# RhushabhVaghela/Custom-NVComp-with-ZSTD

Hardware: AMD Instinct MI355X
Metric: compress GB/s + ratio, 1 GB @ level 3, 64 KB chunks; libzstd round-trip OK (higher is better)
Workload: dtype u8; 1 GPU; C3: 16384 x 64 KiB chunks (1.00 GiB), level 3, independent frames; chunk_bytes=65536, chunks_total=16384, chunks_rank0=16384, level=3, parallelism=dp1 (contiguous chunk shards, RCCL all-gather of sizes inside the step), gathered_frame_bytes=388747049

## Files before the change

### custom-nvcomp-with-zstd_amd/csrc/zh_common.h

```cpp
#pragma once
#include <hip/hip_runtime.h>
#include <stdint.h>
#include "zstd_hip_params.h"
#include "zh_dict_ent.h"
#include "zh_block_plan.h"

typedef int16_t s16;
typedef int32_t s32;

#define ZH_STATS_LIT 0u
#define ZH_STATS_LL 256u
#define ZH_STATS_OF 320u
#define ZH_STATS_ML 384u
#define ZH_STATS_WORDS 448u

#define ZH_SEQ_CAP 13120u
#define ZH_SEQ_BYTES (ZH_SEQ_CAP * 8u)
#define ZH_K3_W 1u
#define ZH_K3_SEGS (21u * ZH_K3_W)
#define ZH_K3_SLOTS (64u * ZH_K3_W)
#define ZH_K3_RUN 16u
#define ZH_K3_SLOT(t, g) (3u * (g) + (t))
#define ZH_K3_TSTRIDE ZH_K3_RUN
#define ZH_K3_SEGLEN(nbseq) ((((nbseq) + ZH_K3_SEGS - 1u) / ZH_K3_SEGS + ZH_K3_RUN - 1u) & ~(ZH_K3_RUN - 1u))
#define ZH_K3_CODES(L) (2u * ZH_K3_SLOTS * (L))
#define ZH_K3_BYTES(nbseq) (3u * ZH_K3_SLOTS * ZH_K3_SEGLEN(nbseq))
#define ZH_LIT_BYTES (ZH_K3_BYTES(ZH_SEQ_CAP) > (u32)ZH_BLOCK_MAX ? ZH_K3_BYTES(ZH_SEQ_CAP) : (u32)ZH_BLOCK_MAX)
static_assert(3u * ZH_K3_SEGS <= ZH_K3_SLOTS, "one lane per (table, segment)");
#define ZH_META_BYTES 256u
#define ZH_FSE_BYTES 4096u
#define ZH_FSE_TAB_BYTES 3528u
#define ZH_FSE_FIELDS 3840u
static_assert(ZH_DENT_FSE_BYTES == ZH_FSE_TAB_BYTES, "the dictionary blob holds the tables in the hand-off layout");
#define ZH_WS_BLOCK_BYTES (ZH_SEQ_BYTES + ZH_LIT_BYTES + ZH_META_BYTES + ZH_FSE_BYTES)
enum : u32 {
  ZH_FT_STLL = 0, ZH_FT_STOF = 1024, ZH_FT_STML = 1536, ZH_FT_SYLL = 2560, ZH_FT_SYOF = 2848, ZH_FT_SYML = 3104,
  ZH_FF_NEED = 0,
  ZH_FF_NBSEQ = 1,
  ZH_FF_OP = 2,
  ZH_FF_BLK = 3,
  ZH_FF_LOGS = 4,
  ZH_FF_SLL = 5, ZH_FF_SOF = 6, ZH_FF_SML = 7,
};

#define ZH_DEEP_STG_BYTES (2u * ZH_BLOCK_MAX + 256u)
#define ZH_DEEP_SLOT_BYTES ((size_t)ZH_DEEP_STG_BYTES + 4u * 2u * ZH_BLOCK_MAX + 4u * ZH_BLOCK_MAX + 2u * 2u * ZH_BLOCK_MAX)
#define ZH_DEEP_SLOTS_MAX 256u
#define ZH_META_K1HIST 2u
#define ZH_K1_HIST_OFF 65536u
#define ZH_K1_HIST_WAVES 16u
static_assert(ZH_K1_HIST_OFF + ZH_K1_HIST_WAVES * 1024u <= ZH_LIT_BYTES, "K1 sub-histograms fit the literal area");

struct ZhWorkspace {
  u8 *base;
  u32 *ctr;
  const u16 *dtab;
  u32 dtab_P;
  const u32 *dd_prev;
  const u32 *dd_head;
  u32 dd_pre, dd_split;
  u8 *deep_slots;
  u32 deep_nslots;
  const ZhDictEnt *dent;
  u32 *stats;
  __device__ u64 *seq(u32 b) const { return (u64 *)(base + (size_t)b * ZH_WS_BLOCK_BYTES); }
  __device__ u8 *lits(u32 b) const { return base + (size_t)b * ZH_WS_BLOCK_BYTES + ZH_SEQ_BYTES; }
  __device__ u32 *meta(u32 b) const { return (u32 *)(base + (size_t)b * ZH_WS_BLOCK_BYTES + ZH_SEQ_BYTES + ZH_LIT_BYTES); }
  __device__ u32 *dbg(u32 b) const { return meta(b) + 4; }
  __device__ u8 *fse(u32 b) const { return base + (size_t)b * ZH_WS_BLOCK_BYTES + ZH_SEQ_BYTES + ZH_LIT_BYTES + ZH_META_BYTES; }
  __device__ u32 *fsef(u32 b) const { return (u32 *)(fse(b) + ZH_FSE_FIELDS); }
};

#define ZH_DTAB_MARGIN 256u

struct ZhClassRanges {
  u32 range[ZH_NCLASSES][2];
  u32 ctr[4];
};
#define ZH_RANGE_CTR_DEEP 3u

__host__ __device__ __forceinline__ u32 zh_k3_magic(u32 L) { return ((1u << 24) + L - 1u) / L; }
__device__ __forceinline__ u32 zh_k3_index(u32 e, u32 t, u32 L, u32 m) {
  u32 const g = __umulhi(e << 8, m), r = e - g * L;
  return ((r / ZH_K3_RUN) * ZH_K3_SLOTS + ZH_K3_SLOT(t, g)) * ZH_K3_RUN + (r & (ZH_K3_RUN - 1u));
}

#define ZH_DPP(v, ctrl, rmask) ((u32)__builtin_amdgcn_update_dpp(0, (int)(v), (ctrl), (rmask), 0xf, false))
__device__ __forceinline__ u32 wave_scan_incl(u32 v) {
  v += ZH_DPP(v, 0x111, 0xf);
  v += ZH_DPP(v, 0x112, 0xf);
  v += ZH_DPP(v, 0x114, 0xf);
  v += ZH_DPP(v, 0x118, 0xf);
  v += ZH_DPP(v, 0x142, 0xa);
  v += ZH_DPP(v, 0x143, 0xc);
  return v;
}
__device__ __forceinline__ u32 wave_scan_max_incl(u32 v) {
  v = max(v, ZH_DPP(v, 0x111, 0xf));
  v = max(v, ZH_DPP(v, 0x112, 0xf));
  v = max(v, ZH_DPP(v, 0x114, 0xf));
  v = max(v, ZH_DPP(v, 0x118, 0xf));
  v = max(v, ZH_DPP(v, 0x142, 0xa));
  v = max(v, ZH_DPP(v, 0x143, 0xc));
  return v;
}
__device__ __forceinline__ u32 wave_shr1(u32 v) { return ZH_DPP(v, 0x138, 0xf); }
__device__ __forceinline__ u32 wave_shl1(u32 v) { return ZH_DPP(v, 0x130, 0xf); }
__device__ __forceinline__ u32 lane_value(u32 v, u32 uniform_lane) { return (u32)__builtin_amdgcn_readlane((int)v, (int)uniform_lane); }
```

### custom-nvcomp-with-zstd_amd/csrc/zh_entropy.hip

```cpp
#include "zh_common.h"

namespace {

constexpr u32 K2_THREADS = 128;
constexpr u32 SW_WORDS = 184;

constexpr u32 OFF_SW = 0;
constexpr u32 OFF_HVAL = OFF_SW + 4 * SW_WORDS;
constexpr u32 OFF_HNB = OFF_HVAL + 2 * 256;
constexpr u32 OFF_MISC = OFF_HNB + 256;
constexpr u32 OFF_HIST = OFF_MISC + 4 * 64;
constexpr u32 OFF_HBUF = OFF_HIST + 4 * 256;
constexpr u32 OFF_SCR = OFF_HBUF + 768;
constexpr u32 OFF_U = OFF_SCR + 1024;
static_assert(OFF_U % 16 == 0, "alignment");
constexpr u32 OFF_NODES = OFF_U;
constexpr u32 U_HUF_END = OFF_NODES + 8 * 516;
constexpr u32 OFF_ST_LL = OFF_U;
constexpr u32 OFF_ST_OF = OFF_ST_LL + 1024;
constexpr u32 OFF_ST_ML = OFF_ST_OF + 512;
constexpr u32 OFF_SYM = OFF_ST_ML + 1024;
constexpr u32 SYM_OF = 36, SYM_ML = 68;
constexpr u32 OFF_TSYM = OFF_SYM + 976;
constexpr u32 OFF_NORM = OFF_TSYM + 512;
// ... 1278 lines not shown
          auto fse_candidate = [&](int &nv) {
            u32 nb1 = nbSeq;
            u32 const tl = fse_optimal_table_log(fseLog, nbSeq, mx, 2);
            u32 const lc = last_code[t];
            if (lane_value(c, lc) > 1) {
              if (lane == lc) c--;
              nb1--;
            }
            nv = fse_normalize_wave(norm, tl, c, nb1, mx, nb1 >= 2048, lane, scr->cumul);
            bmax = mx; blog = tl;
            return fse_write_ncount_wave(hbuf + hposw, nv, mx, tl, lane);
          };
          u32 fse_hs = 0;
          bool fse_done = false;
          if (dent && type != 1) {
            u32 const c0 = c, big = 0xFFFFFFFFu;
            u32 const dc = dent->cost[t][lane];
            u32 const costRep = __ballot(c0 != 0 && dc >= ZH_DENT_IMPOSSIBLE) ? big : wave_sum(c0 * dc);
            u32 costDef = big, costFse = big;
            if (defAllowed) costDef = wave_sum(c0 * fse_cost8(lane <= defMax ? (int)defNorm[lane] : 0, defLog));
            if (mostFrequent < nbSeq) {
              int nv;
              fse_hs = fse_candidate(nv);
              fse_done = true;
              if (fse_hs) costFse = (fse_hs << (3 + ZH_DENT_COST_SHIFT)) + wave_sum(c0 * fse_cost8(nv, blog));
            }
            if (costRep != big && costRep <= costDef && costRep <= costFse) type = 3;
            else if (costDef <= costFse) type = costDef != big ? 0 : type;
            else type = 2;
          }
          if (type == 3) {
            u32 const so = t == 0 ? ZH_FT_STLL : t == 1 ? ZH_FT_STOF : ZH_FT_STML, yo = t == 0 ? ZH_FT_SYLL : t == 1 ? ZH_FT_SYOF : ZH_FT_SYML;
            const u32 *const src = (const u32 *)(dent->fse + so);
            for (u32 i = lane; i < (t == 1 ? 128u : 256u); i += 64) ((u32 *)st)[i] = src[i];
            if (lane <= maxSym) sy[lane] = ((const FseSym *)(dent->fse + yo))[lane];
            logsw[t] = dent->logs[t];
          } else if (type == 1) {
            u32 const fc = first_code[t];
            if (lane == 0) {
              st[0] = 0; st[1] = 0;
              sy[fc].dNb = 0; sy[fc].dFS = 0;
              hbuf[hposw] = (u8)fc;
            }
            hposw++;
            logsw[t] = 0;
          } else if (type == 0) {
            if (lane <= defMax) norm[lane] = defNorm[lane];
            bmax = defMax; blog = defLog;
            logsw[t] = defLog;
          } else {
            int nv;
            if (!fse_done) fse_hs = fse_candidate(nv);
            hposw += fse_hs;
            logsw[t] = blog;
          }
          typesw |= type << (6 - 2 * t);
          wave_sync();
          if (type == 0 || type == 2) fse_build_ctable_par(st, sy, tsym, norm, bmax, blog, scr);
          wave_sync();
        }
        if (lane == 0) {
          misc[0] = hposw;
          misc[1] = typesw;
          misc[2] = logsw[0]; misc[3] = logsw[1]; misc[4] = logsw[2];
        }
      }
      wave_sync();
      hpos = misc[0];
      typesw_ = misc[1];
      logLL = misc[2]; logOF = misc[3]; logML = misc[4];
      ZH_STAMP(6);

      u8 *fz = ws.fse(b);
      {
        const u32 *sL = (const u32 *)stLL, *sO = (const u32 *)stOF, *sM = (const u32 *)stML;
        for (u32 i = lane; i < 256; i += 64) ((u32 *)(fz + ZH_FT_STLL))[i] = sL[i];
        for (u32 i = lane; i < 128; i += 64) ((u32 *)(fz + ZH_FT_STOF))[i] = sO[i];
        for (u32 i = lane; i < 256; i += 64) ((u32 *)(fz + ZH_FT_STML))[i] = sM[i];
        if (lane < 36) ((FseSym *)(fz + ZH_FT_SYLL))[lane] = symLL[lane];
        if (lane < 32) ((FseSym *)(fz + ZH_FT_SYOF))[lane] = symOF[lane];
        if (lane < 53) ((FseSym *)(fz + ZH_FT_SYML))[lane] = symML[lane];
      }
    }
    if (wave == 1 && lane == 0) xch[2] = nbSeq;
    }
    __syncthreads();
    if (xch[1] != 0) {
      u32 const h = (n / 2) & ~63u;
      if (wave == 0) copy_bytes(o, body0, d.src, h);
      else copy_bytes(o, body0 + h, d.src + h, n - h);
    } else if (u32 const ns = xch[2]; ns > 0) {
      u32 const k3L = ZH_K3_SEGLEN(ns), k3m = zh_k3_magic(k3L);
      u8 *const cb = ws.lits(b) + ZH_K3_CODES(k3L);
      for (u32 k0 = 16u * (lane + 64u * wave); k0 < ns; k0 += 16u * K2_THREADS) {
        u64 r[16];
#pragma unroll
        for (u32 q = 0; q < 16; q++) r[q] = k0 + q < ns ? seq[ns - 1 - (k0 + q)] : 0ull;
        u32 wl[4] = {0, 0, 0, 0}, wo[4] = {0, 0, 0, 0}, wm[4] = {0, 0, 0, 0};
#pragma unroll
        for (u32 q = 0; q < 16; q++) {
          u32 const ob = (u32)(r[q] >> 34) & 0x1FFFFu;
          wl[q >> 2] |= ((u32)(r[q] >> 51) & 63u) << (8 * (q & 3));
          wo[q >> 2] |= (ob ? highbit32(ob) : 0u) << (8 * (q & 3));
          wm[q >> 2] |= ((u32)(r[q] >> 57)) << (8 * (q & 3));
        }
        u32 const x0 = zh_k3_index(k0, 0, k3L, k3m);
        *(uint4 *)(cb + x0) = make_uint4(wl[0], wl[1], wl[2], wl[3]);
        *(uint4 *)(cb + x0 + ZH_K3_TSTRIDE) = make_uint4(wo[0], wo[1], wo[2], wo[3]);
        *(uint4 *)(cb + x0 + 2u * ZH_K3_TSTRIDE) = make_uint4(wm[0], wm[1], wm[2], wm[3]);
      }
    }
    if (wave == 1) {
      op = xch[0];
      early_raw = xch[1] != 0;
      if (!early_raw) {
        if (nbSeq < 128) { if (lane == 0) o.put(op, (u8)nbSeq); op += 1; }
        else if (nbSeq < ZH_LONGNBSEQ) { if (lane == 0) { o.put(op, (u8)((nbSeq >> 8) + 0x80)); o.put(op + 1, (u8)nbSeq); } op += 2; }
        else { if (lane == 0) { o.put(op, 0xFF); o.put(op + 1, (u8)(nbSeq - ZH_LONGNBSEQ)); o.put(op + 2, (u8)((nbSeq - ZH_LONGNBSEQ) >> 8)); } op += 3; }
        if (nbSeq > 0) {
          if (lane == 0) o.put(op, (u8)typesw_);
          op += 1;
          for (u32 i = lane; i < hpos; i += 64) o.put(op + i, hbuf[i]);
          op += hpos;
          u32 *ff = ws.fsef(b);
          if (lane == 0) {
            ff[ZH_FF_NBSEQ] = nbSeq; ff[ZH_FF_OP] = op; ff[ZH_FF_BLK] = blk;
            ff[ZH_FF_LOGS] = logLL | (logOF << 8) | (logML << 16);
            ff[ZH_FF_NEED] = 1;
          }
          handoff = true;
        }
      }
      if (early_raw) {
        u32 const hdr = last + (n << 3);
        if (lane == 0) { o.put(blk, (u8)hdr); o.put(blk + 1, (u8)(hdr >> 8)); o.put(blk + 2, (u8)(hdr >> 16)); }
        total = body0 + n;
      } else if (!handoff) {
        total = finish_block(d, o, blk, op, false);
      }
    }
  }
  ZH_STAMP(8);
#ifdef ZH_STAMPS
  if (lane == 0) {
    u32 *dbg = ws.dbg(b);
    if (wave == 0) { for (int k = 0; k < 4; k++) dbg[6 + k] = st[k]; dbg[42] = st[11]; }
    else { for (int k = 4; k < 9; k++) dbg[6 + k] = st[k]; dbg[17] = st[9]; dbg[18] = st[10]; dbg[19] = nseq_raw; }
  }
#endif
  if (wave == 1 && !handoff) write_status(d, b, total, item_size, item_status, blk_size);
}

constexpr u32 K3_SEGS = ZH_K3_SEGS;
constexpr u32 K3_W = ZH_K3_W;
constexpr u32 K3_OCC = 8;
constexpr u32 K3_WARM = 128;
constexpr u32 K3_WAVES = K3_W == 1 ? 4 : K3_W;
constexpr u32 K3_BPW = K3_WAVES / K3_W;
constexpr u32 K3_TAB_STRIDE = (ZH_FSE_TAB_BYTES + 15) & ~15u;
constexpr u32 K3_LDS = K3_BPW * K3_TAB_STRIDE + 64;
constexpr u32 K3_BATCH = 16;
constexpr u32 K3_TABW = ZH_FSE_TAB_BYTES / 4;

__device__ __forceinline__ void k3_chain(ZhWorkspace ws, u32 bb, u8 *smem, u32 lane, u32 *xw) {
#ifdef ZH_STAMPS
  u64 const k3pre = __builtin_amdgcn_s_memtime();
  u64 const k3rt0 = __builtin_amdgcn_s_memrealtime();
#endif
  u32 *ff = ws.fsef(bb);
  {
    const u32 *src = (const u32 *)ws.fse(bb);
    constexpr u32 NT = 64 * K3_W;
    u32 v[(K3_TABW + NT - 1) / NT];
#pragma unroll
    for (u32 q = 0; q < (K3_TABW + NT - 1) / NT; q++) v[q] = NT * q + lane < K3_TABW ? src[NT * q + lane] : 0u;
#pragma unroll
    for (u32 q = 0; q < (K3_TABW + NT - 1) / NT; q++)
      if (NT * q + lane < K3_TABW) ((u32 *)smem)[NT * q + lane] = v[q];
  }
  if constexpr (K3_W == 1) {
    __builtin_amdgcn_fence(__ATOMIC_SEQ_CST, "wavefront");
    __builtin_amdgcn_wave_barrier();
  } else {
    __syncthreads();
  }
  u32 const t = min(lane / K3_SEGS, 2u), g = lane - K3_SEGS * t;
  u32 const nbSeq = ff[ZH_FF_NBSEQ];
  const u16 *stT = (const u16 *)(smem + (t == 0 ? ZH_FT_STLL : t == 1 ? ZH_FT_STOF : ZH_FT_STML));
  const FseSym *syT = (const FseSym *)(smem + (t == 0 ? ZH_FT_SYLL : t == 1 ? ZH_FT_SYOF : ZH_FT_SYML));
  u32 const seglen = ZH_K3_SEGLEN(nbSeq), nk = seglen / K3_BATCH;
  u16 *const gst = (u16 *)ws.lits(bb);
  const u8 *const cbase = ws.lits(bb) + ZH_K3_CODES(seglen);
  u32 const ln = lane < 3 * K3_SEGS ? ZH_K3_SLOT(t, g) : lane, lnp = ZH_K3_SLOT(t, g - 1u);
  auto at = [&](u32 k, u32 slot) { return ((k * K3_BATCH / ZH_K3_RUN) * ZH_K3_SLOTS + slot) * ZH_K3_RUN + (k * K3_BATCH) % ZH_K3_RUN; };
  auto codes_at = [&](u32 k, u32 slot) { return *(const uint4 *)(cbase + at(k, slot)); };
  u32 const a = lane < 3 * K3_SEGS ? g * seglen : 3u * K3_SEGS * seglen;
  auto init_state = [&](u32 code) {
    FseSym const tr = syT[code];
    u32 const nb = (tr.dNb + (1u << 15)) >> 16;
    return (u32)stT[(((nb << 16) - tr.dNb) >> nb) + tr.dFS];
  };
  auto step = [&](u32 s, u32 code, bool live) {
    FseSym const tr = syT[code];
    u32 const nb = (s + tr.dNb) >> 16;
    u32 const nx = stT[min((s >> nb) + (u32)tr.dFS, 1023u)];
    return live ? nx : s;
  };
  u32 entry;
  if (a == 0) {
    entry = init_state(codes_at(0, ln).x & 63u);
  } else {
    constexpr u32 NW = K3_WARM / K3_BATCH;
    constexpr u32 CH = NW < 8u ? NW : 8u;
    static_assert(NW % CH == 0, "warm-up groups");
    u32 const kw = nk > NW ? nk - NW : 0u, ep = a - seglen;
    u32 s = stT[0];
#pragma unroll
    for (u32 j0 = 0; j0 < NW; j0 += CH) {
      uint4 cw[CH];
#pragma unroll
      for (u32 j = 0; j < CH; j++) cw[j] = kw + j0 + j < nk ? codes_at(kw + j0 + j, lnp) : make_uint4(0, 0, 0, 0);
#pragma unroll
      for (u32 j = 0; j < CH; j++) {
        u32 const w[4] = {cw[j].x, cw[j].y, cw[j].z, cw[j].w};
#pragma unroll
        for (u32 q = 0; q < K3_BATCH; q++) {
          u32 const e = ep + K3_BATCH * (kw + j0 + j) + q;
          s = step(s, (w[q >> 2] >> (8 * (q & 3))) & 63u, kw + j0 + j < nk && e >= 1 && e < nbSeq);
        }
      }
    }
    entry = s;
  }
#ifdef ZH_STAMPS
  u64 const k3t0 = __builtin_amdgcn_s_memtime();
  u32 k3rounds = 0, k3rerun = 0;
#endif
  auto pass = [&](u32 &s, bool check) {
    uint4 cn = codes_at(0, ln);
    u32 on = check ? (u32)gst[at(0, ln)] : 0u;
    for (u32 k = 0; k < nk; k++) {
      uint4 const c4 = cn;
      u32 const o = on;
      if (k + 1 < nk) {
        cn = codes_at(k + 1, ln);
        if (check) on = gst[at(k + 1, ln)];
      }
      if (check && s == o) return true;
      u32 const w[4] = {c4.x, c4.y, c4.z, c4.w};
      u32 sv[K3_BATCH];
#pragma unroll
      for (u32 q = 0; q < K3_BATCH; q++) {
        sv[q] = s;
        u32 const e = a + K3_BATCH * k + q;
        s = step(s, (w[q >> 2] >> (8 * (q & 3))) & 63u, e >= 1 && e < nbSeq);
      }
      uint4 *dst = (uint4 *)(gst + at(k, ln));
      dst[0] = make_uint4(sv[0] | (sv[1] << 16), sv[2] | (sv[3] << 16), sv[4] | (sv[5] << 16), sv[6] | (sv[7] << 16));
      dst[1] = make_uint4(sv[8] | (sv[9] << 16), sv[10] | (sv[11] << 16), sv[12] | (sv[13] << 16), sv[14] | (sv[15] << 16));
    }
    return false;
  };
  u32 x = entry;
  (void)pass(x, false);
  for (;;) {
    u32 pe = wave_shr1(x);
    if constexpr (K3_W > 1) {
      if ((lane & 63u) == 63u) xw[lane >> 6] = x;
      __syncthreads();
      if ((lane & 63u) == 0u && lane) pe = xw[(lane >> 6) - 1u];
    }
    u32 const ne = (g == 0 || lane >= 3 * K3_SEGS) ? entry : pe;
    bool const active = ne != entry;
    if constexpr (K3_W > 1) {
      if (__ballot(active) && (lane & 63u) == 0u) atomicOr(&xw[K3_W], 1u);
      __syncthreads();
      bool const any = xw[K3_W] != 0u;
      __syncthreads();
      if (lane == 0) xw[K3_W] = 0u;
      if (!any) break;
    } else {
      if (!__ballot(active)) break;
    }
#ifdef ZH_STAMPS
    k3rounds++;
    k3rerun += __builtin_popcountll(__ballot(active));
#endif
    if (active) {
      entry = ne;
      u32 s = ne;
      if (!pass(s, true)) x = s;
    }
  }
  if (g == K3_SEGS - 1 && lane < 3 * K3_SEGS) ff[ZH_FF_SLL + t] = x;
#ifdef ZH_STAMPS
  if (lane == 0) { u32 *dbg = ws.dbg(bb); dbg[46] = (u32)(__builtin_amdgcn_s_memtime() - k3t0); dbg[47] = k3rounds; dbg[48] = k3rerun; dbg[49] = nbSeq;
                   dbg[50] = (u32)(k3t0 - k3pre); dbg[51] = (u32)k3rt0; dbg[52] = (u32)__builtin_amdgcn_s_memrealtime(); }
#endif
}

extern "C" __global__ __launch_bounds__(64 * K3_WAVES) __attribute__((amdgpu_waves_per_eu(K3_OCC, 8))) void zh_fse_chain_kernel(const ZhBlockDesc *__restrict__ blocks, u32 nblocks, ZhWorkspace ws) {
  extern __shared__ __attribute__((aligned(16))) u8 smem_all[];
  u32 const bw = threadIdx.x / (64 * K3_W), lane = threadIdx.x % (64 * K3_W);
  u32 const bb = blockIdx.x * K3_BPW + bw;
  if (bb >= nblocks || blocks[bb].n == 0) return;
  if (ws.fsef(bb)[ZH_FF_NEED] == 0) return;
  k3_chain(ws, bb, smem_all + bw * K3_TAB_STRIDE, lane, (u32 *)(smem_all + K3_BPW * K3_TAB_STRIDE));
}

constexpr u32 KP_SW = 0, KP_DNB = 4 * SW_WORDS, KP_LDS = (KP_DNB + 4 * 128 + 15) & ~15u;
constexpr u32 K4_WAVES = 4;
constexpr u32 K4_PF = 1;

__device__ __forceinline__ void k4_pack(const ZhBlockDesc &d, ZhWorkspace ws, u32 b, u8 *smem, u32 lane, u64 *__restrict__ item_size,
                                        u32 *__restrict__ item_status, u32 *__restrict__ blk_size) {
  const u32 *ff = ws.fsef(b);
  u32 *sw = (u32 *)(smem + KP_SW);
  u32 *dNb = (u32 *)(smem + KP_DNB);
  const u8 *fz = ws.fse(b);
  if (lane < 36) dNb[lane] = ((const FseSym *)(fz + ZH_FT_SYLL))[lane].dNb;
  if (lane < 32) dNb[40 + lane] = ((const FseSym *)(fz + ZH_FT_SYOF))[lane].dNb;
  if (lane < 53) dNb[72 + lane] = ((const FseSym *)(fz + ZH_FT_SYML))[lane].dNb;
  if (lane == 0) sw[0] = 0;
  u32 const nbSeq = ff[ZH_FF_NBSEQ], logs = ff[ZH_FF_LOGS], blk = ff[ZH_FF_BLK];
  u32 const logLL = logs & 255u, logOF = (logs >> 8) & 255u, logML = logs >> 16;
  u32 const sLL = ff[ZH_FF_SLL], sOF = ff[ZH_FF_SOF], sML = ff[ZH_FF_SML];
  Out const o{d.dst, d.dst_cap};
  const u64 *seq = ws.seq(b);
  u32 const k3L = ZH_K3_SEGLEN(nbSeq), k3m = zh_k3_magic(k3L);
  const u16 *gLL = (const u16 *)ws.lits(b), *gOF = gLL + ZH_K3_TSTRIDE, *gML = gOF + ZH_K3_TSTRIDE;
  CodeTabs ct;
  ct.load();
  wave_sync();
  BitSink bs{ff[ZH_FF_OP], 0};
  u64 rq[K4_PF];
  u32 lq[K4_PF], mq[K4_PF], oq[K4_PF];
  auto fetch = [&](u32 e, u64 &r, u32 &sl, u32 &sm, u32 &so) {
    r = e < nbSeq ? seq[nbSeq - 1 - e] : 0;
    sl = sm = so = 0;
    if (0 < e && e < nbSeq) {
      u32 const x = zh_k3_index(e, 0, k3L, k3m);
      sl = gLL[x]; sm = gML[x]; so = gOF[x];
    }
  };
#pragma unroll
  for (u32 j = 0; j < K4_PF; j++) fetch(64 * j + lane, rq[j], lq[j], mq[j], oq[j]);
  for (u32 e0 = 0; e0 < nbSeq; e0 += 64) {
    u32 const e = e0 + lane;
    bool const valid = e < nbSeq;
    u64 const rec = rq[0];
    u32 const s_L = lq[0], s_M = mq[0], s_O = oq[0];
#pragma unroll
    for (u32 j = 0; j + 1 < K4_PF; j++) { rq[j] = rq[j + 1]; lq[j] = lq[j + 1]; mq[j] = mq[j + 1]; oq[j] = oq[j + 1]; }
    fetch(e + 64 * K4_PF, rq[K4_PF - 1], lq[K4_PF - 1], mq[K4_PF - 1], oq[K4_PF - 1]);
    u32 const ll = (u32)(rec & 0x1FFFFu), mlb = (u32)((rec >> 17) & 0x1FFFFu), ob = (u32)(rec >> 34) & 0x1FFFFu;
    u32 const llc = valid ? (u32)(rec >> 51) & 63u : 0, mlc = valid ? (u32)(rec >> 57) & 63u : 0, ofc = valid ? highbit32(ob) : 0;
    u32 const llbits = ct.ll_bits(llc), mlbits = ct.ml_bits(mlc);
    u32 vOF = 0, nOF = 0, vML = 0, nML = 0, vLL = 0, nLL = 0;
    if (valid && e > 0) {
      nOF = (s_O + dNb[40 + ofc]) >> 16; vOF = s_O;
      nML = (s_M + dNb[72 + mlc]) >> 16; vML = s_M;
      nLL = (s_L + dNb[llc]) >> 16; vLL = s_L;
    }
    u32 v6[6] = {vOF, vML, vLL, ll, mlb, ob};
    u32 n6[6] = {nOF, nML, nLL, valid ? llbits : 0u, valid ? mlbits : 0u, ofc};
    sink_append<6>(bs, o, sw, v6, n6);
  }
  {
    u32 v3[3] = {sML, sOF, sLL};
    u32 n3[3] = {lane == 0 ? logML : 0u, lane == 0 ? logOF : 0u, lane == 0 ? logLL : 0u};
    sink_append<3>(bs, o, sw, v3, n3);
  }
  sink_close(bs, o, sw);
  u32 const total = finish_block(d, o, blk, bs.pos, false);
  write_status(d, b, total, item_size, item_status, blk_size);
}

extern "C" __global__ __launch_bounds__(64 * K4_WAVES) void zh_seq_pack_kernel(const ZhBlockDesc *__restrict__ blocks, u32 nblocks, ZhWorkspace ws,
                                                                               u64 *__restrict__ item_size, u32 *__restrict__ item_status,
                                                                               u32 *__restrict__ blk_size) {
  extern __shared__ __attribute__((aligned(16))) u8 smem_all[];
  u32 const wv = threadIdx.x >> 6, b = blockIdx.x * K4_WAVES + wv;
  if (b >= nblocks) return;
  ZhBlockDesc const d = blocks[b];
  if (d.n == 0 || ws.fsef(b)[ZH_FF_NEED] == 0) return;
  k4_pack(d, ws, b, smem_all + wv * KP_LDS, lane_id(), item_size, item_status, blk_size);
}

extern "C" u32 zh_entropy_lds_bytes() { return K2_LDS; }
#ifdef ZH_STAMPS
extern "C" __global__ void zh_read_hst(u32 *out) { for (int k = 0; k < 6; k++) { out[k] = g_hst[k]; g_hst[k] = 0; } }
extern "C" void zh_hst_host(u32 *out6) {
  u32 *d = nullptr;
  if (hipMalloc(&d, 24) != hipSuccess) return;
  hipLaunchKernelGGL(zh_read_hst, dim3(1), dim3(1), 0, 0, d);
  (void)hipMemcpy(out6, d, 24, hipMemcpyDeviceToHost);
  (void)hipFree(d);
}
#endif

namespace zh {
hipError_t entropy_init() {
  hipError_t e = hipFuncSetAttribute((const void *)zh_entropy_kernel, hipFuncAttributeMaxDynamicSharedMemorySize, (int)K2_LDS);
  if (e == hipSuccess) e = hipFuncSetAttribute((const void *)zh_fse_chain_kernel, hipFuncAttributeMaxDynamicSharedMemorySize, (int)K3_LDS);
  return e;
}
void entropy_launch(const ZhBlockDesc *d_descs, u32 nblocks, ZhWorkspace ws, u32 window_log, u32 cfg_block_size, u64 *d_item_size,
                    u32 *d_item_status, u32 *d_blk_size, const u8 *d_blk_level, hipStream_t stream) {
  hipLaunchKernelGGL(zh_entropy_kernel, dim3(nblocks), dim3(K2_THREADS), K2_LDS, stream, d_descs, ws, window_log, cfg_block_size, d_item_size,
                     d_item_status, d_blk_size, d_blk_level);
  u32 const g3 = (nblocks + K3_BPW - 1) / K3_BPW, g4 = (nblocks + K4_WAVES - 1) / K4_WAVES;
  hipLaunchKernelGGL(zh_fse_chain_kernel, dim3(g3), dim3(64 * K3_WAVES), K3_LDS, stream, d_descs, nblocks, ws);
  hipLaunchKernelGGL(zh_seq_pack_kernel, dim3(g4), dim3(64 * K4_WAVES), K4_WAVES * KP_LDS, stream, d_descs, nblocks, ws, d_item_size,
                     d_item_status, d_blk_size);
}
}
```

Baseline: 91.37 GB/s.

## Fuse FSE chain and sequence pack into one per-block stream kernel

Merges the FSE state-chain kernel and the sequence bitstream pack kernel into a single kernel in which one wave per block runs the chains and then emits the bitstream. Per-sequence states are no longer written out. The chain pass instead stores one start state plus a bit count per 16-sequence batch, and an extra pass precomputes extra-bit totals per batch. This lets each lane emit a whole batch at a known bit offset, with byte boundaries stitched by a segmented OR scan. It removes one launch and the large u16 state array round-trip through global memory, in exchange for recomputing FSE transitions during emission and more complex bit-offset bookkeeping.

```diff
diff --git a/custom-nvcomp-with-zstd_amd/csrc/zh_common.h b/custom-nvcomp-with-zstd_amd/csrc/zh_common.h
--- a/custom-nvcomp-with-zstd_amd/csrc/zh_common.h
+++ b/custom-nvcomp-with-zstd_amd/csrc/zh_common.h
@@ -24,6 +24,7 @@
 #define ZH_K3_TSTRIDE ZH_K3_RUN
 #define ZH_K3_SEGLEN(nbseq) ((((nbseq) + ZH_K3_SEGS - 1u) / ZH_K3_SEGS + ZH_K3_RUN - 1u) & ~(ZH_K3_RUN - 1u))
 #define ZH_K3_CODES(L) (2u * ZH_K3_SLOTS * (L))
+#define ZH_K3_BW(B, t) (4u * (B) + (t))
 #define ZH_K3_BYTES(nbseq) (3u * ZH_K3_SLOTS * ZH_K3_SEGLEN(nbseq))
 #define ZH_LIT_BYTES (ZH_K3_BYTES(ZH_SEQ_CAP) > (u32)ZH_BLOCK_MAX ? ZH_K3_BYTES(ZH_SEQ_CAP) : (u32)ZH_BLOCK_MAX)
 static_assert(3u * ZH_K3_SEGS <= ZH_K3_SLOTS, "one lane per (table, segment)");
@@ -40,7 +41,6 @@
   ZH_FF_OP = 2,
   ZH_FF_BLK = 3,
   ZH_FF_LOGS = 4,
-  ZH_FF_SLL = 5, ZH_FF_SOF = 6, ZH_FF_SML = 7,
 };
 
 #define ZH_DEEP_STG_BYTES (2u * ZH_BLOCK_MAX + 256u)
diff --git a/custom-nvcomp-with-zstd_amd/csrc/zh_entropy.hip b/custom-nvcomp-with-zstd_amd/csrc/zh_entropy.hip
--- a/custom-nvcomp-with-zstd_amd/csrc/zh_entropy.hip
+++ b/custom-nvcomp-with-zstd_amd/csrc/zh_entropy.hip
@@ -1454,44 +1454,60 @@
 }
 
 constexpr u32 K3_SEGS = ZH_K3_SEGS;
-constexpr u32 K3_W = ZH_K3_W;
+static_assert(ZH_K3_W == 1u, "one wave runs a block's chains and packs its bitstream");
 constexpr u32 K3_OCC = 8;
 constexpr u32 K3_WARM = 128;
-constexpr u32 K3_WAVES = K3_W == 1 ? 4 : K3_W;
-constexpr u32 K3_BPW = K3_WAVES / K3_W;
-constexpr u32 K3_TAB_STRIDE = (ZH_FSE_TAB_BYTES + 15) & ~15u;
-constexpr u32 K3_LDS = K3_BPW * K3_TAB_STRIDE + 64;
+constexpr u32 K3_WAVES = 4;
 constexpr u32 K3_BATCH = 16;
+static_assert(K3_BATCH == ZH_K3_RUN, "a batch is one run of the chain layout");
+constexpr u32 K3_RG = 8;
+static_assert(K3_BATCH % K3_RG == 0, "record groups");
 constexpr u32 K3_TABW = ZH_FSE_TAB_BYTES / 4;
-
-__device__ __forceinline__ void k3_chain(ZhWorkspace ws, u32 bb, u8 *smem, u32 lane, u32 *xw) {
+constexpr u32 K3_XB = (ZH_FSE_TAB_BYTES + 15) & ~15u, K3_XB_ML = 64, K3_XB_BYTES = 128;
+constexpr u32 K3_TAB_STRIDE = K3_XB + K3_XB_BYTES;
+constexpr u32 K3_LDS = K3_WAVES * K3_TAB_STRIDE;
+static_assert(K3_XB_ML + 64 <= K3_XB_BYTES && K3_TAB_STRIDE % 16 == 0 && ZH_K3_TSTRIDE == ZH_K3_RUN, "extra-bit rows; a step's three runs");
+
+__device__ __forceinline__ void k3_load_tables(ZhWorkspace ws, u32 bb, u8 *smem, u32 lane) {
+  const u32 *src = (const u32 *)ws.fse(bb);
+  u32 v[(K3_TABW + 63) / 64];
+#pragma unroll
+  for (u32 q = 0; q < (K3_TABW + 63) / 64; q++) v[q] = 64 * q + lane < K3_TABW ? src[64 * q + lane] : 0u;
+#pragma unroll
+  for (u32 q = 0; q < (K3_TABW + 63) / 64; q++)
+    if (64 * q + lane < K3_TABW) ((u32 *)smem)[64 * q + lane] = v[q];
+  u8 *xb = smem + K3_XB;
+  xb[lane] = lane < 36 ? c_LL_bits[lane] : 0;
+  xb[K3_XB_ML + lane] = lane < 53 ? c_ML_bits[lane] : 0;
+  wave_sync();
+}
+
+__device__ __forceinline__ void k3_extra_bits(ZhWorkspace ws, u32 bb, const u8 *smem, u32 lane, u32 nbSeq) {
+  u32 const seglen = ZH_K3_SEGLEN(nbSeq), m = zh_k3_magic(seglen), nbat = (nbSeq + K3_BATCH - 1) / K3_BATCH;
+  const u8 *const cbase = ws.lits(bb) + ZH_K3_CODES(seglen), *xb = smem + K3_XB;
+  u32 *const gbw = (u32 *)ws.lits(bb);
+  for (u32 B = lane; B < nbat; B += 64) {
+    const uint4 *c = (const uint4 *)(cbase + zh_k3_index(K3_BATCH * B, 0, seglen, m));
+    uint4 const cl = c[0], co = c[1], cm = c[2];
+    u32 x = __builtin_amdgcn_sad_u8(co.x, 0u, __builtin_amdgcn_sad_u8(co.y, 0u, __builtin_amdgcn_sad_u8(co.z, 0u, __builtin_amdgcn_sad_u8(co.w, 0u, 0u))));
+    u32 const wl[4] = {cl.x, cl.y, cl.z, cl.w}, wm[4] = {cm.x, cm.y, cm.z, cm.w};
+#pragma unroll
+    for (u32 q = 0; q < K3_BATCH; q++)
+      x += (u32)xb[(wl[q >> 2] >> (8 * (q & 3))) & 63u] + (u32)xb[K3_XB_ML + ((wm[q >> 2] >> (8 * (q & 3))) & 63u)];
+    gbw[ZH_K3_BW(B, 3)] = x;
+  }
+}
+
+__device__ __forceinline__ u32 k3_chain(ZhWorkspace ws, u32 bb, const u8 *smem, u32 lane, u32 nbSeq) {
 #ifdef ZH_STAMPS
   u64 const k3pre = __builtin_amdgcn_s_memtime();
   u64 const k3rt0 = __builtin_amdgcn_s_memrealtime();
 #endif
-  u32 *ff = ws.fsef(bb);
-  {
-    const u32 *src = (const u32 *)ws.fse(bb);
-    constexpr u32 NT = 64 * K3_W;
-    u32 v[(K3_TABW + NT - 1) / NT];
-#pragma unroll
-    for (u32 q = 0; q < (K3_TABW + NT - 1) / NT; q++) v[q] = NT * q + lane < K3_TABW ? src[NT * q + lane] : 0u;
-#pragma unroll
-    for (u32 q = 0; q < (K3_TABW + NT - 1) / NT; q++)
-      if (NT * q + lane < K3_TABW) ((u32 *)smem)[NT * q + lane] = v[q];
-  }
-  if constexpr (K3_W == 1) {
-    __builtin_amdgcn_fence(__ATOMIC_SEQ_CST, "wavefront");
-    __builtin_amdgcn_wave_barrier();
-  } else {
-    __syncthreads();
-  }
   u32 const t = min(lane / K3_SEGS, 2u), g = lane - K3_SEGS * t;
-  u32 const nbSeq = ff[ZH_FF_NBSEQ];
   const u16 *stT = (const u16 *)(smem + (t == 0 ? ZH_FT_STLL : t == 1 ? ZH_FT_STOF : ZH_FT_STML));
   const FseSym *syT = (const FseSym *)(smem + (t == 0 ? ZH_FT_SYLL : t == 1 ? ZH_FT_SYOF : ZH_FT_SYML));
   u32 const seglen = ZH_K3_SEGLEN(nbSeq), nk = seglen / K3_BATCH;
-  u16 *const gst = (u16 *)ws.lits(bb);
+  u32 *const gbw = (u32 *)ws.lits(bb) + ZH_K3_BW(g * nk, t);
   const u8 *const cbase = ws.lits(bb) + ZH_K3_CODES(seglen);
   u32 const ln = lane < 3 * K3_SEGS ? ZH_K3_SLOT(t, g) : lane, lnp = ZH_K3_SLOT(t, g - 1u);
   auto at = [&](u32 k, u32 slot) { return ((k * K3_BATCH / ZH_K3_RUN) * ZH_K3_SLOTS + slot) * ZH_K3_RUN + (k * K3_BATCH) % ZH_K3_RUN; };
@@ -1540,50 +1556,39 @@
 #endif
   auto pass = [&](u32 &s, bool check) {
     uint4 cn = codes_at(0, ln);
-    u32 on = check ? (u32)gst[at(0, ln)] : 0u;
+    u32 on = check ? gbw[0] : 0u;
     for (u32 k = 0; k < nk; k++) {
       uint4 const c4 = cn;
       u32 const o = on;
       if (k + 1 < nk) {
         cn = codes_at(k + 1, ln);
-        if (check) on = gst[at(k + 1, ln)];
-      }
-      if (check && s == o) return true;
+        if (check) on = gbw[ZH_K3_BW(k + 1, 0)];
+      }
+      if (check && s == (o & 0xFFFFu)) return true;
       u32 const w[4] = {c4.x, c4.y, c4.z, c4.w};
-      u32 sv[K3_BATCH];
+      u32 const s0 = s;
+      u32 bits = 0;
 #pragma unroll
       for (u32 q = 0; q < K3_BATCH; q++) {
-        sv[q] = s;
-        u32 const e = a + K3_BATCH * k + q;
-        s = step(s, (w[q >> 2] >> (8 * (q & 3))) & 63u, e >= 1 && e < nbSeq);
-      }
-      uint4 *dst = (uint4 *)(gst + at(k, ln));
-      dst[0] = make_uint4(sv[0] | (sv[1] << 16), sv[2] | (sv[3] << 16), sv[4] | (sv[5] << 16), sv[6] | (sv[7] << 16));
-      dst[1] = make_uint4(sv[8] | (sv[9] << 16), sv[10] | (sv[11] << 16), sv[12] | (sv[13] << 16), sv[14] | (sv[15] << 16));
+        u32 const e = a + K3_BATCH * k + q, code = (w[q >> 2] >> (8 * (q & 3))) & 63u;
+        FseSym const tr = syT[code];
+        u32 const nb = (s + tr.dNb) >> 16;
+        u32 const nx = stT[min((s >> nb) + (u32)tr.dFS, 1023u)];
+        bool const live = (q > 0 || e >= 1) && e < nbSeq;
+        bits += live ? nb : 0u;
+        s = live ? nx : s;
+      }
+      gbw[ZH_K3_BW(k, 0)] = s0 | (bits << 16);
     }
     return false;
   };
   u32 x = entry;
   (void)pass(x, false);
   for (;;) {
-    u32 pe = wave_shr1(x);
-    if constexpr (K3_W > 1) {
-      if ((lane & 63u) == 63u) xw[lane >> 6] = x;
-      __syncthreads();
-      if ((lane & 63u) == 0u && lane) pe = xw[(lane >> 6) - 1u];
-    }
+    u32 const pe = wave_shr1(x);
     u32 const ne = (g == 0 || lane >= 3 * K3_SEGS) ? entry : pe;
     bool const active = ne != entry;
-    if constexpr (K3_W > 1) {
-      if (__ballot(active) && (lane & 63u) == 0u) atomicOr(&xw[K3_W], 1u);
-      __syncthreads();
-      bool const any = xw[K3_W] != 0u;
-      __syncthreads();
-      if (lane == 0) xw[K3_W] = 0u;
-      if (!any) break;
-    } else {
-      if (!__ballot(active)) break;
-    }
+    if (!__ballot(active)) break;
 #ifdef ZH_STAMPS
     k3rounds++;
     k3rerun += __builtin_popcountll(__ballot(active));
@@ -1594,99 +1599,167 @@
       if (!pass(s, true)) x = s;
     }
   }
-  if (g == K3_SEGS - 1 && lane < 3 * K3_SEGS) ff[ZH_FF_SLL + t] = x;
 #ifdef ZH_STAMPS
   if (lane == 0) { u32 *dbg = ws.dbg(bb); dbg[46] = (u32)(__builtin_amdgcn_s_memtime() - k3t0); dbg[47] = k3rounds; dbg[48] = k3rerun; dbg[49] = nbSeq;
-                   dbg[50] = (u32)(k3t0 - k3pre); dbg[51] = (u32)k3rt0; dbg[52] = (u32)__builtin_amdgcn_s_memrealtime(); }
+                   dbg[50] = (u32)(k3t0 - k3pre); dbg[51] = (u32)k3rt0; }
 #endif
-}
-
-extern "C" __global__ __launch_bounds__(64 * K3_WAVES) __attribute__((amdgpu_waves_per_eu(K3_OCC, 8))) void zh_fse_chain_kernel(const ZhBlockDesc *__restrict__ blocks, u32 nblocks, ZhWorkspace ws) {
+  return x;
+}
+
+__device__ __forceinline__ u32 wave_segscan_or(u32 v) {
+  auto run = [](u32 left, u32 right) { return (right & 0x100u) ? right : (left | right); };
+  v = run(ZH_DPP(v, 0x111, 0xf), v);
+  v = run(ZH_DPP(v, 0x112, 0xf), v);
+  v = run(ZH_DPP(v, 0x114, 0xf), v);
+  v = run(ZH_DPP(v, 0x118, 0xf), v);
+  v = run(ZH_DPP(v, 0x142, 0xa), v);
+  v = run(ZH_DPP(v, 0x143, 0xc), v);
+  return v;
+}
+
+struct alignas(16) RecPair { u64 a, b; };
+
+__device__ __forceinline__ u32 k3_emit(ZhWorkspace ws, u32 bb, const u8 *smem, u32 lane, u32 nbSeq, const Out &o, u32 op, u32 logs, u32 sLL,
+                                       u32 sOF, u32 sML) {
+  const u16 *stLL = (const u16 *)(smem + ZH_FT_STLL), *stOF = (const u16 *)(smem + ZH_FT_STOF), *stML = (const u16 *)(smem + ZH_FT_STML);
+  const FseSym *syLL = (const FseSym *)(smem + ZH_FT_SYLL), *syOF = (const FseSym *)(smem + ZH_FT_SYOF),
+               *syML = (const FseSym *)(smem + ZH_FT_SYML);
+  const u8 *xb = smem + K3_XB;
+  const uint4 *gbw = (const uint4 *)ws.lits(bb);
+  const RecPair *seq2 = (const RecPair *)ws.seq(bb);
+  u32 const nbat = (nbSeq + K3_BATCH - 1) / K3_BATCH;
+  auto put_tail = [&](u32 pos, u64 v, u32 cnt) {
+    if (cnt >= 4u) {
+      u32 const wd = (u32)v;
+      if (pos + 4u <= o.cap) __builtin_memcpy(o.dst + pos, &wd, 4);
+      v >>= 32; pos += 4u; cnt -= 4u;
+    }
+#pragma unroll
+    for (u32 i = 0; i < 3; i++)
+      if (i < cnt) o.put(pos + i, (u8)(v >> (8 * i)));
+  };
+  bool const odd = nbSeq & 1u;
+  u32 rel = 0;
+  u32 cprev = 0;
+  for (u32 b0 = 0; b0 < nbat; b0 += 64) {
+    u32 const B = b0 + lane;
+    uint4 const w = B < nbat ? gbw[B] : make_uint4(0, 0, 0, 0);
+    u64 r[K3_RG];
+    auto load_records = [&](u32 q0) {
+      s32 const A = (s32)nbSeq - (s32)K3_RG - (s32)(K3_BATCH * B + q0) - (s32)odd;
+      RecPair pr[K3_RG / 2 + 1];
+#pragma unroll
+      for (u32 p = 0; p < K3_RG / 2 + 1; p++) {
+        s32 const i = A + 2 * (s32)p;
+        pr[p] = (i >= 0 && i < (s32)ZH_SEQ_CAP && (p < K3_RG / 2 || odd)) ? seq2[i >> 1] : RecPair{0ull, 0ull};
+      }
+#pragma unroll
+      for (u32 q = 0; q < K3_RG; q++) {
+        u32 const k = K3_RG - 1 - q;
+        u64 const even = (k & 1u) ? pr[k >> 1].b : pr[k >> 1].a, other = (k & 1u) ? pr[(k + 1) >> 1].a : pr[(k + 1) >> 1].b;
+        r[q] = K3_BATCH * B + q0 + q < nbSeq ? (odd ? other : even) : 0ull;
+      }
+    };
+    load_records(0);
+    u32 const T = (w.x >> 16) + (w.y >> 16) + (w.z >> 16) + w.w;
+    u32 tot;
+    u32 const bit0 = rel + wave_excl_scan(T, tot);
+    u32 const pos0 = op + (bit0 >> 3);
+    bool const roomy = op + ((rel + tot) >> 3) + 1u <= o.cap;
+    u32 sL = w.x & 0xFFFFu, sO = w.y & 0xFFFFu, sM = w.z & 0xFFFFu;
+    u64 lo = 0, hi = 0;
+    u32 n = bit0 & 7u, pos = pos0, w0 = 0;
+    auto append = [&](u64 v, u32 nb) {
+      lo |= v << n;
+      hi |= (v >> 1) >> (63u - n);
+      n += nb;
+      if (n >= 64u) {
+        w0 = pos == pos0 ? (u32)lo : w0;
+        if (roomy) __builtin_memcpy(o.dst + pos, &lo, 8);
+        pos += 8u;
+        lo = hi; hi = 0;
+        n -= 64u;
+      }
+    };
+    for (u32 q0 = 0; q0 < K3_BATCH; q0 += K3_RG) {
+      if (q0) load_records(q0);
+#pragma unroll
+      for (u32 q = 0; q < K3_RG; q++) {
+        u32 const e = K3_BATCH * B + q0 + q;
+        bool const live = (q > 0 || e >= 1) && e < nbSeq;
+        u64 const rec = r[q];
+        u32 const ll = (u32)rec & 0x1FFFFu, mlb = (u32)(rec >> 17) & 0x1FFFFu, ob = (u32)(rec >> 34) & 0x1FFFFu;
+        u32 const llc = (u32)(rec >> 51) & 63u, mlc = (u32)(rec >> 57) & 63u, ofc = ob ? highbit32(ob) : 0u;
+        FseSym const tO = syOF[ofc], tM = syML[mlc], tL = syLL[llc];
+        u32 const nO = live ? (sO + tO.dNb) >> 16 : 0u, nM = live ? (sM + tM.dNb) >> 16 : 0u, nL = live ? (sL + tL.dNb) >> 16 : 0u;
+        u32 const llx = xb[llc], mlx = xb[K3_XB_ML + mlc], ns = nO + nM + nL;
+        u32 const c1 = __builtin_amdgcn_ubfe(sO, 0u, nO) | (__builtin_amdgcn_ubfe(sM, 0u, nM) << nO) | (__builtin_amdgcn_ubfe(sL, 0u, nL) << (nO + nM));
+        u32 const c2 = __builtin_amdgcn_ubfe(ll, 0u, llx) | (__builtin_amdgcn_ubfe(mlb, 0u, mlx) << llx);
+        u32 const n12 = ns + llx + mlx, c3 = __builtin_amdgcn_ubfe(ob, 0u, ofc);
+        u64 const v12 = c1 | ((u64)c2 << ns);
+        if (__ballot(n12 + ofc > 64u) == 0) {
+          append(v12 | ((u64)c3 << n12), n12 + ofc);
+        } else {
+          append(v12, n12);
+          append(c3, ofc);
+        }
+        u32 const xO = stOF[min((sO >> nO) + (u32)tO.dFS, 1023u)], xM = stML[min((sM >> nM) + (u32)tM.dFS, 1023u)],
+                  xL = stLL[min((sL >> nL) + (u32)tL.dFS, 1023u)];
+        sO = live ? xO : sO; sM = live ? xM : sM; sL = live ? xL : sL;
+      }
+    }
+    bool const filled = pos != pos0;
+    u32 const nfull = n >> 3;
+    bool const reset = filled || nfull != 0u;
+    u32 own = (u32)(lo >> (8u * nfull)) & 0xFFu;
+    if (lane == 0 && !reset) own |= cprev;
+    u32 const c = wave_segscan_or(own | (reset ? 0x100u : 0u));
+    u32 const left = wave_shr1(c) & 0xFFu;
+    u32 const cin = lane == 0 ? cprev : left;
+    cprev = lane_value(c, 63) & 0xFFu;
+    if (filled && cin) o.put(pos0, (u8)(w0 | cin));
+    put_tail(pos, filled ? lo : lo | cin, nfull);
+    rel += tot;
+  }
+  u32 const logLL = logs & 255u, logOF = (logs >> 8) & 255u, logML = logs >> 16;
+  u64 fa = cprev;
+  u32 fn = rel & 7u;
+  fa |= (u64)__builtin_amdgcn_ubfe(sML, 0u, logML) << fn; fn += logML;
+  fa |= (u64)__builtin_amdgcn_ubfe(sOF, 0u, logOF) << fn; fn += logOF;
+  fa |= (u64)__builtin_amdgcn_ubfe(sLL, 0u, logLL) << fn; fn += logLL;
+  fa |= 1ull << fn; fn += 1u;
+  u32 const fpos = op + (rel >> 3), fbytes = (fn + 7u) >> 3;
+  if (lane < fbytes) o.put(fpos + lane, (u8)(fa >> (8u * lane)));
+  return fpos + fbytes;
+}
+
+extern "C" __global__ __launch_bounds__(64 * K3_WAVES) __attribute__((amdgpu_waves_per_eu(K3_OCC, 8))) void zh_seq_stream_kernel(
+    const ZhBlockDesc *__restrict__ blocks, u32 nblocks, ZhWorkspace ws, u64 *__restrict__ item_size, u32 *__restrict__ item_status,
+    u32 *__restrict__ blk_size) {
   extern __shared__ __attribute__((aligned(16))) u8 smem_all[];
-  u32 const bw = threadIdx.x / (64 * K3_W), lane = threadIdx.x % (64 * K3_W);
-  u32 const bb = blockIdx.x * K3_BPW + bw;
-  if (bb >= nblocks || blocks[bb].n == 0) return;
-  if (ws.fsef(bb)[ZH_FF_NEED] == 0) return;
-  k3_chain(ws, bb, smem_all + bw * K3_TAB_STRIDE, lane, (u32 *)(smem_all + K3_BPW * K3_TAB_STRIDE));
-}
-
-constexpr u32 KP_SW = 0, KP_DNB = 4 * SW_WORDS, KP_LDS = (KP_DNB + 4 * 128 + 15) & ~15u;
-constexpr u32 K4_WAVES = 4;
-constexpr u32 K4_PF = 1;
-
-__device__ __forceinline__ void k4_pack(const ZhBlockDesc &d, ZhWorkspace ws, u32 b, u8 *smem, u32 lane, u64 *__restrict__ item_size,
-                                        u32 *__restrict__ item_status, u32 *__restrict__ blk_size) {
-  const u32 *ff = ws.fsef(b);
-  u32 *sw = (u32 *)(smem + KP_SW);
-  u32 *dNb = (u32 *)(smem + KP_DNB);
-  const u8 *fz = ws.fse(b);
-  if (lane < 36) dNb[lane] = ((const FseSym *)(fz + ZH_FT_SYLL))[lane].dNb;
-  if (lane < 32) dNb[40 + lane] = ((const FseSym *)(fz + ZH_FT_SYOF))[lane].dNb;
-  if (lane < 53) dNb[72 + lane] = ((const FseSym *)(fz + ZH_FT_SYML))[lane].dNb;
-  if (lane == 0) sw[0] = 0;
-  u32 const nbSeq = ff[ZH_FF_NBSEQ], logs = ff[ZH_FF_LOGS], blk = ff[ZH_FF_BLK];
-  u32 const logLL = logs & 255u, logOF = (logs >> 8) & 255u, logML = logs >> 16;
-  u32 const sLL = ff[ZH_FF_SLL], sOF = ff[ZH_FF_SOF], sML = ff[ZH_FF_SML];
+  u32 const wv = (u32)__builtin_amdgcn_readfirstlane((int)(threadIdx.x >> 6)), lane = lane_id(), bb = blockIdx.x * K3_WAVES + wv;
+  if (bb >= nblocks) return;
+  ZhBlockDesc const d = blocks[bb];
+  const u32 *ff = ws.fsef(bb);
+  if (d.n == 0 || ff[ZH_FF_NEED] == 0) return;
+  u8 *const smem = smem_all + wv * K3_TAB_STRIDE;
+  k3_load_tables(ws, bb, smem, lane);
+  u32 const nbSeq = ff[ZH_FF_NBSEQ], logs = ff[ZH_FF_LOGS], blk = ff[ZH_FF_BLK], op = ff[ZH_FF_OP];
+  k3_extra_bits(ws, bb, smem, lane, nbSeq);
+  u32 const x = k3_chain(ws, bb, smem, lane, nbSeq);
+  __builtin_amdgcn_fence(__ATOMIC_SEQ_CST, "workgroup");
+  __builtin_amdgcn_wave_barrier();
+#ifdef ZH_STAMPS
+  u64 const k3e0 = __builtin_amdgcn_s_memtime();
+#endif
   Out const o{d.dst, d.dst_cap};
-  const u64 *seq = ws.seq(b);
-  u32 const k3L = ZH_K3_SEGLEN(nbSeq), k3m = zh_k3_magic(k3L);
-  const u16 *gLL = (const u16 *)ws.lits(b), *gOF = gLL + ZH_K3_TSTRIDE, *gML = gOF + ZH_K3_TSTRIDE;
-  CodeTabs ct;
-  ct.load();
-  wave_sync();
-  BitSink bs{ff[ZH_FF_OP], 0};
-  u64 rq[K4_PF];
-  u32 lq[K4_PF], mq[K4_PF], oq[K4_PF];
-  auto fetch = [&](u32 e, u64 &r, u32 &sl, u32 &sm, u32 &so) {
-    r = e < nbSeq ? seq[nbSeq - 1 - e] : 0;
-    sl = sm = so = 0;
-    if (0 < e && e < nbSeq) {
-      u32 const x = zh_k3_index(e, 0, k3L, k3m);
-      sl = gLL[x]; sm = gML[x]; so = gOF[x];
-    }
-  };
-#pragma unroll
-  for (u32 j = 0; j < K4_PF; j++) fetch(64 * j + lane, rq[j], lq[j], mq[j], oq[j]);
-  for (u32 e0 = 0; e0 < nbSeq; e0 += 64) {
-    u32 const e = e0 + lane;
-    bool const valid = e < nbSeq;
-    u64 const rec = rq[0];
-    u32 const s_L = lq[0], s_M = mq[0], s_O = oq[0];
-#pragma unroll
-    for (u32 j = 0; j + 1 < K4_PF; j++) { rq[j] = rq[j + 1]; lq[j] = lq[j + 1]; mq[j] = mq[j + 1]; oq[j] = oq[j + 1]; }
-    fetch(e + 64 * K4_PF, rq[K4_PF - 1], lq[K4_PF - 1], mq[K4_PF - 1], oq[K4_PF - 1]);
-    u32 const ll = (u32)(rec & 0x1FFFFu), mlb = (u32)((rec >> 17) & 0x1FFFFu), ob = (u32)(rec >> 34) & 0x1FFFFu;
-    u32 const llc = valid ? (u32)(rec >> 51) & 63u : 0, mlc = valid ? (u32)(rec >> 57) & 63u : 0, ofc = valid ? highbit32(ob) : 0;
-    u32 const llbits = ct.ll_bits(llc), mlbits = ct.ml_bits(mlc);
-    u32 vOF = 0, nOF = 0, vML = 0, nML = 0, vLL = 0, nLL = 0;
-    if (valid && e > 0) {
-      nOF = (s_O + dNb[40 + ofc]) >> 16; vOF = s_O;
-      nML = (s_M + dNb[72 + mlc]) >> 16; vML = s_M;
-      nLL = (s_L + dNb[llc]) >> 16; vLL = s_L;
-    }
-    u32 v6[6] = {vOF, vML, vLL, ll, mlb, ob};
-    u32 n6[6] = {nOF, nML, nLL, valid ? llbits : 0u, valid ? mlbits : 0u, ofc};
-    sink_append<6>(bs, o, sw, v6, n6);
-  }
-  {
-    u32 v3[3] = {sML, sOF, sLL};
-    u32 n3[3] = {lane == 0 ? logML : 0u, lane == 0 ? logOF : 0u, lane == 0 ? logLL : 0u};
-    sink_append<3>(bs, o, sw, v3, n3);
-  }
-  sink_close(bs, o, sw);
-  u32 const total = finish_block(d, o, blk, bs.pos, false);
-  write_status(d, b, total, item_size, item_status, blk_size);
-}
-
-extern "C" __global__ __launch_bounds__(64 * K4_WAVES) void zh_seq_pack_kernel(const ZhBlockDesc *__restrict__ blocks, u32 nblocks, ZhWorkspace ws,
-                                                                               u64 *__restrict__ item_size, u32 *__restrict__ item_status,
-                                                                               u32 *__restrict__ blk_size) {
-  extern __shared__ __attribute__((aligned(16))) u8 smem_all[];
-  u32 const wv = threadIdx.x >> 6, b = blockIdx.x * K4_WAVES + wv;
-  if (b >= nblocks) return;
-  ZhBlockDesc const d = blocks[b];
-  if (d.n == 0 || ws.fsef(b)[ZH_FF_NEED] == 0) return;
-  k4_pack(d, ws, b, smem_all + wv * KP_LDS, lane_id(), item_size, item_status, blk_size);
+  u32 const end = k3_emit(ws, bb, smem, lane, nbSeq, o, op, logs, lane_value(x, K3_SEGS - 1), lane_value(x, 2 * K3_SEGS - 1),
+                          lane_value(x, 3 * K3_SEGS - 1));
+#ifdef ZH_STAMPS
+  if (lane == 0) { u32 *dbg = ws.dbg(bb); dbg[53] = (u32)(__builtin_amdgcn_s_memtime() - k3e0); dbg[52] = (u32)__builtin_amdgcn_s_memrealtime(); }
+#endif
+  u32 const total = finish_block(d, o, blk, end, false);
+  write_status(d, bb, total, item_size, item_status, blk_size);
 }
 
 extern "C" u32 zh_entropy_lds_bytes() { return K2_LDS; }
@@ -1704,16 +1777,14 @@
 namespace zh {
 hipError_t entropy_init() {
   hipError_t e = hipFuncSetAttribute((const void *)zh_entropy_kernel, hipFuncAttributeMaxDynamicSharedMemorySize, (int)K2_LDS);
-  if (e == hipSuccess) e = hipFuncSetAttribute((const void *)zh_fse_chain_kernel, hipFuncAttributeMaxDynamicSharedMemorySize, (int)K3_LDS);
+  if (e == hipSuccess) e = hipFuncSetAttribute((const void *)zh_seq_stream_kernel, hipFuncAttributeMaxDynamicSharedMemorySize, (int)K3_LDS);
   return e;
 }
 void entropy_launch(const ZhBlockDesc *d_descs, u32 nblocks, ZhWorkspace ws, u32 window_log, u32 cfg_block_size, u64 *d_item_size,
                     u32 *d_item_status, u32 *d_blk_size, const u8 *d_blk_level, hipStream_t stream) {
   hipLaunchKernelGGL(zh_entropy_kernel, dim3(nblocks), dim3(K2_THREADS), K2_LDS, stream, d_descs, ws, window_log, cfg_block_size, d_item_size,
                      d_item_status, d_blk_size, d_blk_level);
-  u32 const g3 = (nblocks + K3_BPW - 1) / K3_BPW, g4 = (nblocks + K4_WAVES - 1) / K4_WAVES;
-  hipLaunchKernelGGL(zh_fse_chain_kernel, dim3(g3), dim3(64 * K3_WAVES), K3_LDS, stream, d_descs, nblocks, ws);
-  hipLaunchKernelGGL(zh_seq_pack_kernel, dim3(g4), dim3(64 * K4_WAVES), K4_WAVES * KP_LDS, stream, d_descs, nblocks, ws, d_item_size,
-                     d_item_status, d_blk_size);
-}
-}
+  hipLaunchKernelGGL(zh_seq_stream_kernel, dim3((nblocks + K3_WAVES - 1) / K3_WAVES), dim3(64 * K3_WAVES), K3_LDS, stream, d_descs, nblocks,
+                     ws, d_item_size, d_item_status, d_blk_size);
+}
+}
```

After: 92.28 GB/s (median of 6 runs). Within noise of the previous version (+1.0%).
